# hila-chefer/Transformer-Explainability

Measured on NVIDIA H100. Metric: explanations_per_sec, higher is better.
Workload: dtype f32

## Files before the change

### transformer_explainability_b200/csrc/te_tc_wgmma.cu

```cuda
#include <cuda.h>
#include <cuda_bf16.h>
#include <cuda_fp16.h>
#include <cuda_runtime.h>
#include <string.h>
#include <algorithm>
#include <string>
#include <type_traits>
#include <utility>

#include "te_gemm_tc.h"
#include "te_wgmma.cuh"

namespace {

constexpr int BM = 128, NTHREADS = 256;

__device__ __forceinline__ uint32_t smem_u32(const void* p) { return (uint32_t)__cvta_generic_to_shared(p); }
__device__ __forceinline__ void fence_proxy_async() { asm volatile("fence.proxy.async.shared::cta;" ::: "memory"); }
__device__ __forceinline__ void wg_fence() { asm volatile("wgmma.fence.sync.aligned;" ::: "memory"); }
__device__ __forceinline__ void wg_commit() { asm volatile("wgmma.commit_group.sync.aligned;" ::: "memory"); }
__device__ __forceinline__ void wg_wait0() { asm volatile("wgmma.wait_group.sync.aligned 0;" ::: "memory"); }
__device__ __forceinline__ void wg_wait1() { asm volatile("wgmma.wait_group.sync.aligned 1;" ::: "memory"); }

__device__ __forceinline__ void mbar_init(uint32_t bar, uint32_t count) {
    asm volatile("mbarrier.init.shared::cta.b64 [%0], %1;" ::"r"(bar), "r"(count) : "memory");
}
__device__ __forceinline__ void mbar_expect_tx(uint32_t bar, uint32_t bytes) {
    asm volatile("mbarrier.arrive.expect_tx.shared::cta.b64 _, [%0], %1;" ::"r"(bar), "r"(bytes) : "memory");
}
__device__ __forceinline__ void mbar_arrive(uint32_t bar) { asm volatile("mbarrier.arrive.shared::cta.b64 _, [%0];" ::"r"(bar) : "memory"); }
__device__ __forceinline__ void mbar_wait(uint32_t bar, uint32_t parity) {
    uint32_t done;
    do {
        asm volatile("{\n.reg .pred p;\nmbarrier.try_wait.parity.shared::cta.b64 p, [%1], %2;\nselp.u32 %0, 1, 0, p;\n}\n"
                     : "=r"(done) : "r"(bar), "r"(parity) : "memory");
    } while (!done);
}
__device__ __forceinline__ void tma_load(uint32_t dst, const CUtensorMap* map, int k, int row, uint32_t bar) {
    asm volatile("cp.async.bulk.tensor.2d.shared::cluster.global.tile.mbarrier::complete_tx::bytes [%0], [%1, {%2, %3}], [%4];"
                 ::"r"(dst), "l"((uint64_t)map), "r"(k), "r"(row), "r"(bar) : "memory");
}
__device__ __forceinline__ void tma_load3(uint32_t dst, const CUtensorMap* map, int x, int y, int z, uint32_t bar) {
    asm volatile("cp.async.bulk.tensor.3d.shared::cluster.global.tile.mbarrier::complete_tx::bytes [%0], [%1, {%2, %3, %4}], [%5];"
                 ::"r"(dst), "l"((uint64_t)map), "r"(x), "r"(y), "r"(z), "r"(bar) : "memory");
}
__device__ __forceinline__ void bar_named(int id, int threads) { asm volatile("bar.sync %0, %1;" ::"r"(id), "r"(threads) : "memory"); }
template <int N>
__device__ __forceinline__ void setmaxnreg_dec() { asm volatile("setmaxnreg.dec.sync.aligned.u32 %0;" ::"n"(N)); }
template <int N>
__device__ __forceinline__ void setmaxnreg_inc() { asm volatile("setmaxnreg.inc.sync.aligned.u32 %0;" ::"n"(N)); }

__device__ __forceinline__ float to_tf32(float x) {
    uint32_t u;
    asm("cvt.rna.tf32.f32 %0, %1;" : "=r"(u) : "f"(x));
    return __uint_as_float(u);
}
__device__ __forceinline__ float4 tf32x4(float4 v) { return make_float4(to_tf32(v.x), to_tf32(v.y), to_tf32(v.z), to_tf32(v.w)); }
__device__ __forceinline__ float4 absx4(float4 v) { return make_float4(fabsf(v.x), fabsf(v.y), fabsf(v.z), fabsf(v.w)); }
__device__ __forceinline__ float4 posx4(float4 v) { return make_float4(fmaxf(v.x, 0.f), fmaxf(v.y, 0.f), fmaxf(v.z, 0.f), fmaxf(v.w, 0.f)); }
__device__ __forceinline__ float4 negx4(float4 v) { return make_float4(fminf(v.x, 0.f), fminf(v.y, 0.f), fminf(v.z, 0.f), fminf(v.w, 0.f)); }
__device__ __forceinline__ float4 subx4(float4 a, float4 b) { return make_float4(a.x - b.x, a.y - b.y, a.z - b.z, a.w - b.w); }

__device__ __forceinline__ float ex2_approx(float x) {
    float y;
    asm("ex2.approx.ftz.f32 %0, %1;" : "=f"(y) : "f"(x));
    return y;
}

__device__ __forceinline__ uint32_t swz(int r, int c) { return (uint32_t)r * 128u + ((uint32_t)(c ^ (r & 7)) << 4); }

// ... 117 lines not shown
}
template <bool SP>
__device__ __forceinline__ auto put_tf32(uint8_t* hi, uint8_t* lo) {
    return [=](int r, int c, float4 v) {
        if (SP) st4(hi, r, c, tf32x4(v));
        else st_split(hi, lo, r, c, v);
    };
}
template <bool SP>
__device__ __forceinline__ void fix_tf32(uint8_t* hi, uint8_t* lo, int r0, int n, int t, int nt) {
    if (SP) map_rows(hi, r0, n, t, nt, [](float4 v) { return tf32x4(v); });
    else split_rows(hi, lo, r0, n, t, nt);
}

__device__ __forceinline__ int frag_row(int tid, int j) { return 64 * (tid >> 7) + 16 * ((tid >> 5) & 3) + ((tid & 31) >> 2) + 8 * ((j >> 1) & 1); }
__device__ __forceinline__ int frag_col(int tid, int j) { return 8 * (j >> 2) + 2 * (tid & 3) + (j & 1); }

constexpr int TMA_MAPS = 5;
struct TmaArgs {
    CUtensorMap map[TMA_MAPS];
    int mtiles, ntiles, nz;
};
enum { FIX_NONE = 0, FIX_A = 1, FIX_AB = 2 };
constexpr int NTHREADS_TMA = 384, SMEM_MAX = 227 * 1024;
__host__ __device__ constexpr int tma_stages(int bytes, int epi) {
    return (SMEM_MAX - 1024 - 256 - epi) / bytes < 8 ? (SMEM_MAX - 1024 - 256 - epi) / bytes : 8;
}

template <class P>
__host__ __device__ constexpr int epi_bytes() { return P::EPI_MAPS * BM * P::BN * 4; }
__device__ __forceinline__ float2 epi_f2(const uint8_t* t, int r, int c) {
    return *reinterpret_cast<const float2*>(t + (c >> 5) * (BM * 128) + swz(r, (c & 31) >> 2) + (c & 3) * 4);
}

template <class P, int NA, int NR, int NT, int NTR>
__device__ __forceinline__ void fold(const P& p, float (&acc)[NA][NR], float (&tot)[NT][NTR], int m0, int ch, int z, int tid) {
    const float s0 = p.chunk_scale(m0 + frag_row(tid, 0), ch, z), s1 = p.chunk_scale(m0 + frag_row(tid, 2), ch, z);
#pragma unroll
    for (int a = 0; a < NA; ++a)
#pragma unroll
        for (int j = 0; j < NR; ++j) tot[a][j] = fmaf(acc[a][j], ((j >> 1) & 1) ? s1 : s0, tot[a][j]);
}
template <int NA, int NR>
__device__ __forceinline__ void zero(float (&v)[NA][NR]) {
#pragma unroll
    for (int a = 0; a < NA; ++a)
#pragma unroll
        for (int j = 0; j < NR; ++j) v[a][j] = 0.f;
}

template <class P>
__device__ __forceinline__ void reg_tile(const P& p, uint8_t* smem, int col_fast) {
    constexpr int NR = P::BN / 2;
    constexpr int NA = P::PRODS::NACC;
    constexpr int STAGE = P::L::BYTES;
    constexpr int NT = P::CHUNK ? NA : 1, NTR = P::CHUNK ? NR : 1;
    const int tid = threadIdx.x, wg = tid >> 7;
    const int m0 = (col_fast ? blockIdx.y : blockIdx.x) * BM, n0 = (col_fast ? blockIdx.x : blockIdx.y) * P::BN;
    const int z = blockIdx.z;
    float acc[NA][NR];
    float tot[NT][NTR];
    zero(acc);
    zero(tot);

    const int kb = p.kblocks();
    p.load(smem, 0, m0, n0, z, tid);
    fence_proxy_async();
    __syncthreads();
    for (int it = 0; it < kb; ++it) {
        const bool fresh = P::CHUNK ? (it % P::CHUNK == 0) : (it == 0);
        wg_fence();
        issue<P>(smem_u32(smem + (it & 1) * STAGE), wg, acc, fresh ? 0u : 1u);
        wg_commit();
        if (it + 1 < kb) p.load(smem + ((it + 1) & 1) * STAGE, it + 1, m0, n0, z, tid);
        wg_wait0();
        if constexpr (P::CHUNK > 0)
            if ((it + 1) % P::CHUNK == 0 || it + 1 == kb) fold(p, acc, tot, m0, it / P::CHUNK, z, tid);
        fence_proxy_async();
        __syncthreads();
    }
    if constexpr (P::CHUNK > 0) p.epilogue(tot, m0, n0, z, tid, nullptr);
    else p.epilogue(acc, m0, n0, z, tid, nullptr);
}

template <class P>
__device__ __forceinline__ void tma_tiles(const P& p, const TmaArgs& ta, uint8_t* smem) {
    using L = typename P::L;
    constexpr int NR = P::BN / 2;
    constexpr int NA = P::PRODS::NACC;
    constexpr int STAGE = L::BYTES, EPI = epi_bytes<P>(), S = tma_stages(STAGE, EPI);
    constexpr int NT = P::CHUNK ? NA : 1, NTR = P::CHUNK ? NR : 1;
    static_assert(S >= 2, "a TMA problem needs two stages");
    __shared__ __align__(8) uint64_t bars[2 * S + 2];
    const int tid = threadIdx.x, wg = tid >> 7;
    const uint32_t full0 = smem_u32(bars), empty0 = full0 + 8u * S, st0 = smem_u32(smem);
    const uint32_t efull = full0 + 16u * S, eempty = efull + 8u, ebuf = st0 + (uint32_t)S * STAGE;
    if (tid == 0) {
        for (int s = 0; s < S; ++s) {
            mbar_init(full0 + 8u * s, 1);
            mbar_init(empty0 + 8u * s, 8);
        }
        mbar_init(efull, 1);
        mbar_init(eempty, 8);
        asm volatile("fence.mbarrier_init.release.cluster;" ::: "memory");
    }
    __syncthreads();
    const int kb = p.kblocks(), per_z = ta.mtiles * ta.ntiles, ntiles = ta.nz * per_z;
    int stage = 0;
    uint32_t phase = 0;
    auto decode = [&](int t, int& m0, int& n0, int& z) {
        z = t / per_z;
        const int r = t - z * per_z;
        m0 = (r / ta.ntiles) * BM;
        n0 = (r % ta.ntiles) * P::BN;
    };

    if (wg == 2) {
        setmaxnreg_dec<40>();
        if (tid != 2 * 128) return;
        uint32_t ephase = 0;
        for (int t = blockIdx.x; t < ntiles; t += gridDim.x) {
            int m0, n0, z;
            decode(t, m0, n0, z);
            for (int it = 0; it < kb; ++it) {
                mbar_wait(empty0 + 8u * stage, phase ^ 1u);
                p.produce(ta, st0 + (uint32_t)stage * STAGE, full0 + 8u * stage, it, m0, n0, z);
                if (++stage == S) { stage = 0; phase ^= 1u; }
                if constexpr (EPI > 0) {
                    if (it == min(S, kb) - 1) {
                        mbar_wait(eempty, ephase ^ 1u);
                        mbar_expect_tx(efull, EPI);
#pragma unroll
                        for (int i = 0; i < P::EPI_MAPS; ++i)
#pragma unroll
                            for (int b = 0; b < P::BN / 32; ++b)
                                tma_load(ebuf + (uint32_t)(i * BM * P::BN * 4 + b * BM * 128), &ta.map[P::NMAPS + i], n0 + 32 * b,
                                         m0, efull);
                        ephase ^= 1u;
                    }
                }
            }
        }
        return;
    }

    setmaxnreg_inc<232>();
    float acc[NA][NR];
    float tot[NT][NTR];
    auto release = [&](int s) {
        if ((tid & 31) == 0) mbar_arrive(empty0 + 8u * s);
    };
    auto consume = [&](uint32_t sd) {
        mbar_wait(full0 + 8u * stage, phase);
        if constexpr (P::FIX != FIX_NONE) {
            p.fix(smem + (uint32_t)stage * STAGE, wg, tid);
            fence_proxy_async();
            if constexpr (P::FIX == FIX_A) bar_named(1 + wg, 128);
            else bar_named(3, 256);
        }
        wg_fence();
        issue<P>(st0 + (uint32_t)stage * STAGE, wg, acc, sd);
        wg_commit();
    };
    auto next = [&] {
        if (++stage == S) { stage = 0; phase ^= 1u; }
    };
    constexpr int CH = P::CHUNK;
    uint32_t ephase = 0;
    for (int t = blockIdx.x; t < ntiles; t += gridDim.x) {
        int m0, n0, z;
        decode(t, m0, n0, z);
        zero(acc);
        zero(tot);
        for (int k0 = 0; k0 < kb; k0 += CH ? CH : kb) {
            const int k1 = CH ? min(k0 + CH, kb) : kb;
            consume(0u);
            for (int it = k0 + 1; it < k1; ++it) {
                const int prev = stage;
                next();
                consume(1u);
                wg_wait1();
                release(prev);
            }
            wg_wait0();
            release(stage);
            next();
            if constexpr (CH > 0) fold(p, acc, tot, m0, k0 / CH, z, tid);
        }
        if constexpr (EPI > 0) mbar_wait(efull, ephase);
        if constexpr (P::CHUNK > 0) p.epilogue(tot, m0, n0, z, tid, smem + (uint32_t)S * STAGE);
        else p.epilogue(acc, m0, n0, z, tid, smem + (uint32_t)S * STAGE);
        if constexpr (EPI > 0) {
            __syncwarp();
            if ((tid & 31) == 0) mbar_arrive(eempty);
            ephase ^= 1u;
        }
    }
}

template <class P>
__global__ void __launch_bounds__(P::TMA ? NTHREADS_TMA : NTHREADS, 1)
    wg_kernel(const P p, const __grid_constant__ TmaArgs ta, int col_fast) {
    extern __shared__ uint8_t smem_raw[];
    uint8_t* smem = smem_raw + ((1024u - (smem_u32(smem_raw) & 1023u)) & 1023u);
    if constexpr (P::TMA) tma_tiles(p, ta, smem);
    else reg_tile(p, smem, col_fast);
}

struct NoScale {
    __device__ __forceinline__ float chunk_scale(int, int, int) const { return 1.f; }
};

struct TmaTile {
    const void* base;
    long long rows, cols, ld;
    int box_rows;
    long long count = 0, cstride = 0;
};
template <class P>
__device__ __forceinline__ void produce_tiles(const TmaArgs& ta, uint32_t st, uint32_t bar, int it, int m0, int n0) {
    using L = typename P::L;
    constexpr int KE = P::FMT == OP_TF32 ? 32 : 64;
    mbar_expect_tx(bar, L::BYTES);
#pragma unroll
    for (int i = 0; i < L::NTA; ++i) tma_load(st + L::a(i), &ta.map[i], it * KE, m0, bar);
#pragma unroll
    for (int j = 0; j < L::NTB; ++j) tma_load(st + L::b(j), &ta.map[L::NTA + j], it * KE, n0, bar);
}
#define TE_PRODUCE_TILES(P)                                                                                      \
    static constexpr int NMAPS = L::NTA + L::NTB;                                                                \
    __device__ void produce(const TmaArgs& ta, uint32_t st, uint32_t bar, int it, int m0, int n0, int) const { \
        produce_tiles<P>(ta, st, bar, it, m0, n0);                                                               \
    }

enum { ZO_F32 = 0, ZO_BF16 = 1, ZO_F16S = 2 };
template <bool SINGLE, bool BF, int OUT>
struct ZsProb : NoScale {
    static constexpr int BN = 128, CHUNK = 0, FMT = BF ? OP_BF16 : OP_TF32;
    using PRODS = std::conditional_t<SINGLE, One, Prods<Pr<0, 0, 0>, Pr<0, 1, 1>>>;
    using L = Stage<PRODS, BN>;
    static constexpr bool COL_FAST = true;
    static constexpr bool TMA = SINGLE;
    static constexpr int FIX = SINGLE && !BF ? FIX_A : FIX_NONE;
    static constexpr int EPI_MAPS = SINGLE ? 2 : 0;
    int M, N, K;
    const float* x; long long ldx;
    const void* xabs;
    const void* wa; const void* wb;
    const float* r; long long ldr; const float* y; long long ldy; const float* bias;
    void* out; long long ldo; float* hs;
    float sscale, zsign;

    __device__ int kblocks() const { return K / (BF ? 64 : 32); }
    __device__ void fix(uint8_t* st, int wg, int tid) const {
        map_rows(st + L::a(0), 64 * wg, 64, tid & 127, 128, [](float4 v) { return tf32x4(absx4(v)); });
    }
    TE_PRODUCE_TILES(ZsProb)
    TmaTile tile(int i) const {
        if (i == 0) return BF ? TmaTile{xabs, M, K, K, BM} : TmaTile{x, M, K, ldx, BM};
        if (i == 1) return TmaTile{wa, N, K, K, BN};
        return i == 2 ? TmaTile{r, M, N, ldr, BM} : TmaTile{y, M, N, ldy, BM};
    }
    __device__ void load(uint8_t* st, int kb, int m0, int n0, int, int tid) const {
        for_k32(BM, x, ldx, m0, M, kb * 32, K, tid, [&](int rr, int c, float4 v) {
            st4(st + L::a(0), rr, c, tf32x4(posx4(v)));
            st4(st + L::a(1), rr, c, tf32x4(negx4(v)));
        });
        for_k32(BN, (const float*)wa, K, n0, N, kb * 32, K, tid, [&](int rr, int c, float4 v) { st4(st + L::b(0), rr, c, v); });
        for_k32(BN, (const float*)wb, K, n0, N, kb * 32, K, tid, [&](int rr, int c, float4 v) { st4(st + L::b(1), rr, c, v); });
    }
    __device__ void epilogue(float (&acc)[1][BN / 2], int m0, int n0, int, int tid, const uint8_t* eb) const {
        float sv[BN / 2];
        float rmax[2] = {0.f, 0.f};
#pragma unroll
        for (int j = 0; j < BN / 2; j += 2) {
            const int row = m0 + frag_row(tid, j), col = n0 + frag_col(tid, j);
            float2 rr = make_float2(0.f, 0.f), z = make_float2(acc[0][j], acc[0][j + 1]);
            if (row < M) {
                rr = SINGLE ? epi_f2(eb, frag_row(tid, j), frag_col(tid, j))
                            : *reinterpret_cast<const float2*>(r + (long long)row * ldr + col);
                if (SINGLE) {
                    const float2 yy = epi_f2(eb + BM * BN * 4, frag_row(tid, j), frag_col(tid, j));
                    const float2 bb = bias ? *reinterpret_cast<const float2*>(bias + col) : make_float2(0.f, 0.f);
                    z.x = 0.5f * ((yy.x - bb.x) + zsign * z.x);
                    z.y = 0.5f * ((yy.y - bb.y) + zsign * z.y);
                    z = zsign > 0.f ? make_float2(fmaxf(z.x, 0.f), fmaxf(z.y, 0.f)) : make_float2(fminf(z.x, 0.f), fminf(z.y, 0.f));
                }
            }
            sv[j] = sscale * te_sd(rr.x, z.x);
            sv[j + 1] = sscale * te_sd(rr.y, z.y);
            if (OUT == ZO_F16S) rmax[(j >> 1) & 1] = fmaxf(rmax[(j >> 1) & 1], fmaxf(fabsf(sv[j]), fabsf(sv[j + 1])));
        }
#pragma unroll
        for (int j = 0; j < BN / 2; j += 2) {
            const int row = m0 + frag_row(tid, j), col = n0 + frag_col(tid, j);
            if (row >= M) continue;
            if (OUT == ZO_F32) {
                *reinterpret_cast<float2*>((float*)out + (long long)row * ldo + col) = make_float2(to_tf32(sv[j]), to_tf32(sv[j + 1]));
            } else if (OUT == ZO_BF16) {
                *reinterpret_cast<__nv_bfloat162*>((__nv_bfloat16*)out + (long long)row * ldo + col) = __floats2bfloat162_rn(sv[j], sv[j + 1]);
            }
        }
        if (OUT == ZO_F16S) {
            float sc[2];
#pragma unroll
            for (int h = 0; h < 2; ++h) {
                float m = rmax[h];
                m = fmaxf(m, __shfl_xor_sync(0xffffffffu, m, 1));
                m = fmaxf(m, __shfl_xor_sync(0xffffffffu, m, 2));
                float si;
                te_f16_block_scale(m, sc[h], si);
                const int row = m0 + frag_row(tid, 2 * h);
                if ((tid & 3) == 0 && row < M) hs[(long long)row * (N / 128) + n0 / 128] = si;
            }
#pragma unroll
            for (int j = 0; j < BN / 2; j += 2) {
                const int row = m0 + frag_row(tid, j), col = n0 + frag_col(tid, j);
                const float s = sc[(j >> 1) & 1];
                if (row < M) *reinterpret_cast<__half2*>((__half*)out + (long long)row * N + col) = __floats2half2_rn(sv[j] * s, sv[j + 1] * s);
            }
        }
    }
};

template <int KIND>
struct ZrProb {
    static constexpr int BN = (KIND == 2) ? 64 : 128, CHUNK = (KIND == 2) ? 2 : 0;
    static constexpr int FMT = KIND == 0 ? OP_TF32 : KIND == 1 ? OP_BF16 : OP_F16;
    using PRODS = Prods<Pr<0, 0, 0>, Pr<1, 0, 1>>;
    using L = Stage<PRODS, BN>;
    static constexpr bool TMA = true;
    static constexpr int FIX = FIX_NONE, EPI_MAPS = KIND == 0 ? 0 : 1;
    int M, N, K;
    const void* s; const void* wp; const void* wn;
    const float* rs; int rs_ld; const float* cp; const float* cn;
    const float* x; long long ldx; float* out; long long ldo;
    int accum;

    __device__ int kblocks() const { return K / (KIND ? 64 : 32); }
    TE_PRODUCE_TILES(ZrProb)
    __device__ float chunk_scale(int row, int ch, int) const { return (KIND == 2 && row < M) ? rs[(long long)row * rs_ld + ch] : 1.f; }
    TmaTile tile(int i) const {
        if (i == 0) return TmaTile{s, M, K, K, BM};
        return i < 3 ? TmaTile{i == 1 ? wp : wn, N, K, K, BN} : TmaTile{x, M, N, ldx, BM};
    }
    __device__ void epilogue(float (&acc)[2][BN / 2], int m0, int n0, int, int tid, const uint8_t* eb) const {
#pragma unroll
        for (int j = 0; j < BN / 2; j += 2) {
            const int row = m0 + frag_row(tid, j), col = n0 + frag_col(tid, j);
            if (row >= M) continue;
            const float2 xv = EPI_MAPS ? epi_f2(eb, frag_row(tid, j), frag_col(tid, j))
                                       : *reinterpret_cast<const float2*>(x + (long long)row * ldx + col);
            float2 ap = make_float2(acc[0][j], acc[0][j + 1]), an = make_float2(acc[1][j], acc[1][j + 1]);
            if (KIND == 2) {
                ap.x *= cp[col]; ap.y *= cp[col + 1];
                an.x *= cn[col]; an.y *= cn[col + 1];
            }
            float2 v = make_float2(fmaxf(xv.x, 0.f) * ap.x + fminf(xv.x, 0.f) * an.x, fmaxf(xv.y, 0.f) * ap.y + fminf(xv.y, 0.f) * an.y);
            if (accum) {
                const float2 prev = *reinterpret_cast<const float2*>(out + (long long)row * ldo + col);
                v = make_float2(prev.x + v.x, prev.y + v.y);
            }
            acc[0][j] = v.x;
            acc[0][j + 1] = v.y;
        }
// ... 8 lines not shown
template <bool NEG>
struct LrpSProb : NoScale {
    static constexpr int BN = 128, CHUNK = 0, FMT = OP_TF32;
    using PRODS = One;
    using L = Stage<PRODS, BN>;
    static constexpr bool COL_FAST = true, TMA = false;
    int M, N, K;
    const float* x; long long ldx; const float* w;
    const float* r; long long ldr; float* out;
    float sscale;
    __device__ int kblocks() const { return K / 32; }
    __device__ void load(uint8_t* st, int kb, int m0, int n0, int, int tid) const {
        for_k32(BM, x, ldx, m0, M, kb * 32, K, tid, [&](int rr, int c, float4 v) { st4(st + L::a(0), rr, c, tf32x4(NEG ? negx4(v) : posx4(v))); });
        for_k32(BN, w, K, n0, N, kb * 32, K, tid, [&](int rr, int c, float4 v) { st4(st + L::b(0), rr, c, v); });
    }
    __device__ void epilogue(float (&acc)[1][BN / 2], int m0, int n0, int, int tid, const uint8_t*) const {
#pragma unroll
        for (int j = 0; j < BN / 2; j += 2) {
            const int row = m0 + frag_row(tid, j), col = n0 + frag_col(tid, j);
            if (row >= M) continue;
            const float2 rr = *reinterpret_cast<const float2*>(r + (long long)row * ldr + col);
            *reinterpret_cast<float2*>(out + (long long)row * N + col) =
                make_float2(to_tf32(sscale * te_sd(rr.x, acc[0][j])), to_tf32(sscale * te_sd(rr.y, acc[0][j + 1])));
        }
    }
};
template <bool NEG>
struct LrpRProb : NoScale {
    static constexpr int BN = 128, CHUNK = 0, FMT = OP_TF32;
    using PRODS = One;
    using L = Stage<PRODS, BN>;
    static constexpr bool TMA = true;
    static constexpr int FIX = FIX_NONE, EPI_MAPS = 1;
    int M, N, K;
    const float* s; const float* wt;
    const float* x; long long ldx; float* out; long long ldo;
    int accum;
    __device__ int kblocks() const { return K / 32; }
    TE_PRODUCE_TILES(LrpRProb)
    TmaTile tile(int i) const {
        return i == 0 ? TmaTile{s, M, K, K, BM} : i == 1 ? TmaTile{wt, N, K, K, BN} : TmaTile{x, M, N, ldx, BM};
    }
    __device__ void epilogue(float (&acc)[1][BN / 2], int m0, int n0, int, int tid, const uint8_t* eb) const {
#pragma unroll
        for (int j = 0; j < BN / 2; j += 2) {
            const int row = m0 + frag_row(tid, j), col = n0 + frag_col(tid, j);
            if (row >= M) continue;
            const float2 xv = epi_f2(eb, frag_row(tid, j), frag_col(tid, j));
            const float2* o = reinterpret_cast<const float2*>(out + (long long)row * ldo + col);
            float2 v;
            if (NEG) {
                const float2 prev = *o;
                v = make_float2(prev.x + fminf(xv.x, 0.f) * acc[0][j], prev.y + fminf(xv.y, 0.f) * acc[0][j + 1]);
            } else if (accum) {
                const float2 prev = *o;
                v = make_float2(prev.x + fmaxf(xv.x, 0.f) * acc[0][j], prev.y + fmaxf(xv.y, 0.f) * acc[0][j + 1]);
            } else {
                v = make_float2(fmaxf(xv.x, 0.f) * acc[0][j], fmaxf(xv.y, 0.f) * acc[0][j + 1]);
            }
            acc[0][j] = v.x;
            acc[0][j + 1] = v.y;
        }
#pragma unroll
        for (int j = 0; j < BN / 2; j += 2) {
            const int row = m0 + frag_row(tid, j), col = n0 + frag_col(tid, j);
            if (row < M) *reinterpret_cast<float2*>(out + (long long)row * ldo + col) = make_float2(acc[0][j], acc[0][j + 1]);
// ... 20 lines not shown
}
template <int EPI, class EF>
__device__ __forceinline__ void lin_store(const LinOut& o, int row, int col, float2 y, EF e) {
    *reinterpret_cast<float2*>(o.C + (long long)row * o.ldc + col) = y;
    float2 y2 = make_float2(0.f, 0.f);
    if (EPI == TE_TC_EPI_BIAS_GELU) y2 = make_float2(te_gelu(y.x), te_gelu(y.y));
    if (EPI == TE_TC_EPI_BIAS_ADD) {
        const float2 ev = e();
        y2 = make_float2(ev.x + y.x, ev.y + y.y);
    }
    if (EPI == TE_TC_EPI_BIAS_GELU || EPI == TE_TC_EPI_BIAS_ADD) *reinterpret_cast<float2*>(o.C2 + (long long)row * o.ldc2 + col) = y2;
}

enum { LIN_3XTF32 = 0, LIN_TF32 = 1, LIN_F16X3 = 2, LIN_F16 = 3 };
struct LinArgs {
    int K, rs_ld;
    const void* a; const void* a_lo; long long lda;
    const void* b; const void* b_lo;
    const float* rs; const float* cs;
    LinOut o;
};
static_assert(sizeof(LinArgs) <= 128, "LinArgs: keep the kernel parameter within 128 bytes");
template <int EPI, int FORM>
struct LinProb : LinArgs {
    static constexpr bool F16 = FORM == LIN_F16X3 || FORM == LIN_F16, SPLIT = FORM == LIN_3XTF32 || FORM == LIN_F16X3;
    static constexpr int BN = FORM == LIN_TF32 && EPI == TE_TC_EPI_STORE ? 256 : 128;
    static constexpr int CHUNK = F16 ? 2 : SPLIT ? 4 : 0, FMT = F16 ? OP_F16 : OP_TF32;
    using PRODS = std::conditional_t<SPLIT, Split3, One>;
    using L = Stage<PRODS, BN>;
    static constexpr bool COL_FAST = true;
    static constexpr bool TMA = FORM != LIN_3XTF32;
    static constexpr int FIX = FORM == LIN_TF32 ? FIX_A : FIX_NONE;
    static constexpr int EPI_MAPS = TMA && EPI == TE_TC_EPI_GELU_BWD ? 1 : 0;
    __device__ int kblocks() const { return K / (F16 ? 64 : 32); }
    __device__ float chunk_scale(int row, int ch, int) const {
        if constexpr (F16) return row < o.M ? rs[(long long)row * rs_ld + ch] : 1.f;
        else return 1.f;
    }
    __device__ void fix(uint8_t* st, int wg, int tid) const {
        map_rows(st + L::a(0), 64 * wg, 64, tid & 127, 128, [](float4 v) { return tf32x4(v); });
    }
    TE_PRODUCE_TILES(LinProb)
    TmaTile tile(int i) const {
        if (i < L::NTA) return TmaTile{i == 0 ? a : a_lo, o.M, K, F16 ? K : lda, BM};
        if (i < NMAPS) return TmaTile{i == L::NTA ? b : b_lo, o.N, K, K, BN};
        return TmaTile{o.E, o.M, o.N, o.lde, BM};
    }
    __device__ void load(uint8_t* st, int kb, int m0, int n0, int, int tid) const {
        for_k32(BM, (const float*)a, lda, m0, o.M, kb * 32, K, tid, [&](int r, int c, float4 v) { st_split(st + L::a(0), st + L::a(1), r, c, v); });
        for_k32(BN, (const float*)b, K, n0, o.N, kb * 32, K, tid, [&](int r, int c, float4 v) { st4(st + L::b(0), r, c, v); });
        for_k32(BN, (const float*)b_lo, K, n0, o.N, kb * 32, K, tid, [&](int r, int c, float4 v) { st4(st + L::b(1), r, c, v); });
    }
    __device__ void epilogue(float (&acc)[1][BN / 2], int m0, int n0, int, int tid, const uint8_t* eb) const {
        auto inside = [&](int row, int col) { return row < o.M && (BN == 128 || col < o.N); };
        constexpr bool E_FIRST = EPI == TE_TC_EPI_BIAS_ADD && EPI_MAPS == 0;
        float2 ef[E_FIRST ? BN / 4 : 1];
#pragma unroll
        for (int j = 0; j < BN / 2; j += 2) {
            const int row = m0 + frag_row(tid, j), col = n0 + frag_col(tid, j);
            if (!inside(row, col)) continue;
            if constexpr (E_FIRST) ef[j / 2] = efrag(eb, tid, j, row, col);
            auto e = [&] { return efrag(eb, tid, j, row, col); };
            float2 y;
            if constexpr (F16)
                y = lin_value<EPI, false>(o, col, acc[0][j] * cs[col], acc[0][j + 1] * cs[col + 1], e);
            else y = lin_value<EPI, FORM == LIN_TF32>(o, col, acc[0][j], acc[0][j + 1], e);
            acc[0][j] = y.x;
            acc[0][j + 1] = y.y;
        }
#pragma unroll
        for (int j = 0; j < BN / 2; j += 2) {
            const int row = m0 + frag_row(tid, j), col = n0 + frag_col(tid, j);
            if (inside(row, col))
                lin_store<EPI>(o, row, col, make_float2(acc[0][j], acc[0][j + 1]), [&] {
                    if constexpr (E_FIRST) return ef[j / 2];
                    else return efrag(eb, tid, j, row, col);
                });
        }
    }
    __device__ float2 efrag(const uint8_t* eb, int tid, int j, int row, int col) const {
        if constexpr (EPI_MAPS > 0) return epi_f2(eb, frag_row(tid, j), frag_col(tid, j));
        else return *reinterpret_cast<const float2*>(o.E + (long long)row * o.lde + col);
    }
};

enum { AT_STORE = 0, AT_MUL = 1, AT_SD = 2, AT_SOFTMAX = 3, AT_RESID = 4 };
template <int EPI, bool SP, int BN_>
struct NnProb : NoScale {
    static constexpr int BN = BN_, CHUNK = 0, FMT = OP_TF32;
    using PRODS = std::conditional_t<SP, One, Split3>;
    using L = Stage<PRODS, BN>;
    static constexpr bool TMA = true;
    static constexpr int FIX = FIX_AB, EPI_MAPS = 0;
    int N, H, dh, ld_out, batch;
    const float* a; long long lda; const float* b; long long ldb;
    const float* E; float* out; float alpha;
    __device__ int kblocks() const { return dh / 32; }
    static constexpr int NMAPS = 2;
    TmaTile tile(int i) const {
        return i == 0 ? TmaTile{a, (long long)batch * N, H * dh, lda, BM} : TmaTile{b, (long long)batch * N, H * dh, ldb, BN};
    }
    __device__ void produce(const TmaArgs& ta, uint32_t st, uint32_t bar, int kb, int m0, int n0, int bh) const {
        const int s = bh / H, k = (bh % H) * dh + kb * 32;
        mbar_expect_tx(bar, TILE128 + BN * 128);
        tma_load(st + L::a(0), &ta.map[0], k, s * N + m0, bar);
        tma_load(st + L::b(0), &ta.map[1], k, s * N + n0, bar);
    }
    __device__ void fix(uint8_t* st, int wg, int tid) const {
        fix_tf32<SP>(st + L::a(0), st + L::a(1), 64 * wg, 64, tid & 127, 128);
        fix_tf32<SP>(st + L::b(0), st + L::b(1), 0, BN, tid, 256);
    }
    __device__ void epilogue(float (&acc)[1][BN / 2], int m0, int n0, int bh, int tid, const uint8_t*) const {
        const int ncols = (N + 3) & ~3;
        if constexpr (EPI == AT_SOFTMAX) {
            float mx[2] = {-INFINITY, -INFINITY};
#pragma unroll
            for (int j = 0; j < BN / 2; ++j)
                if (n0 + frag_col(tid, j) < N) mx[(j >> 1) & 1] = fmaxf(mx[(j >> 1) & 1], alpha * acc[0][j]);
            float sum[2] = {0.f, 0.f}, m2[2];
#pragma unroll
            for (int h = 0; h < 2; ++h) {
                mx[h] = fmaxf(mx[h], __shfl_xor_sync(0xffffffffu, mx[h], 1));
                mx[h] = fmaxf(mx[h], __shfl_xor_sync(0xffffffffu, mx[h], 2));
                m2[h] = -mx[h] * 1.4426950408889634f;
            }
            const float a2 = alpha * 1.4426950408889634f;
// ... 22 lines not shown
        for (int j = 0; j < BN / 2; j += 2) {
            const int r = m0 + frag_row(tid, j), col = n0 + frag_col(tid, j);
            ef[j / 2] = (EPI != AT_STORE && r < N && col < ncols)
                            ? *reinterpret_cast<const float2*>(E + ((long long)bh * N + r) * ld_out + col) : make_float2(0.f, 0.f);
        }
#pragma unroll
        for (int j = 0; j < BN / 2; j += 2) {
            const int r = m0 + frag_row(tid, j), col = n0 + frag_col(tid, j);
            if (r >= N || col >= ncols) continue;
            const long long off = ((long long)bh * N + r) * ld_out + col;
            const float2 e = ef[j / 2];
            float v[2] = {alpha * acc[0][j], alpha * acc[0][j + 1]};
            const float ee[2] = {e.x, e.y};
#pragma unroll
            for (int u = 0; u < 2; ++u) {
                if (EPI == AT_MUL) v[u] *= ee[u];
                else if (EPI == AT_SD) v[u] = te_sd_fast(ee[u], v[u]);
                if (col + u >= N) v[u] = 0.f;
            }
            *reinterpret_cast<float2*>(out + off) = make_float2(v[0], v[1]);
        }
        }
    }
};

template <int AMN, int EPI, bool SP, int BN_>
struct NkProb : NoScale {
    static constexpr int BN = BN_, CHUNK = SP ? 0 : 4, FMT = OP_TF32;
    using PRODS = std::conditional_t<SP, One, Split3>;
    static constexpr int LAND_A = AMN ? BM * 128 : 0, LAND_X = BN * 128;
    using L = Stage<PRODS, BN, LAND_A + LAND_X>;
    static constexpr bool TMA = true;
    static constexpr int FIX = FIX_AB, EPI_MAPS = 0;
    int N, H, NP, ld_out, n_out, n_pad, a_shared, batch;
    const float* map; const float* X; long long ldx;
    const float* rowscale; const float* E; float* out; float alpha;
    __device__ int kblocks() const { return (N + 31) / 32; }
    static constexpr int NMAPS = 2;
    TmaTile tile(int i) const {
        if (i == 0) return TmaTile{map, N, N, NP, AMN ? 32 : BM, (long long)batch * (a_shared ? 1 : H), (long long)N * NP};
        return TmaTile{X, N, n_pad, ldx, 32, batch, (long long)N * ldx};
    }
    __device__ void produce(const TmaArgs& ta, uint32_t st, uint32_t bar, int kb, int m0, int, int bh) const {
        const int s = bh / H, h = bh % H, za = a_shared ? s : bh;
        mbar_expect_tx(bar, (AMN ? LAND_A : TILE128) + LAND_X);
        if (AMN == 0) tma_load3(st + L::a(0), &ta.map[0], kb * 32, m0, za, bar);
#pragma unroll
        for (int j = 0; j < LAND_A / 4096; ++j) tma_load3(st + L::land() + j * 4096, &ta.map[0], m0 + 32 * j, kb * 32, za, bar);
#pragma unroll
        for (int j = 0; j < LAND_X / 4096; ++j)
            tma_load3(st + L::land() + LAND_A + j * 4096, &ta.map[1], h * BN + 32 * j, kb * 32, s, bar);
    }
    __device__ void fix(uint8_t* st, int wg, int tid) const {
        if (AMN) transpose_rows(st + L::land(), 64 * wg, 64, tid & 127, 128, put_tf32<SP>(st + L::a(0), st + L::a(1)));
        else fix_tf32<SP>(st + L::a(0), st + L::a(1), 64 * wg, 64, tid & 127, 128);
        transpose_rows(st + L::land() + LAND_A, 0, BN, tid, 256, put_tf32<SP>(st + L::b(0), st + L::b(1)));
    }
    __device__ void epilogue(float (&acc)[1][BN / 2], int m0, int, int bh, int tid, const uint8_t*) const {
        const int s = bh / H, h = bh % H;
        float2 ef[BN / 4];
#pragma unroll
        for (int j = 0; j < BN / 2; j += 2) {
            const int m = m0 + frag_row(tid, j), gcol = h * BN + frag_col(tid, j);
            ef[j / 2] = (EPI != AT_STORE && m < N && gcol < n_pad)
                            ? *reinterpret_cast<const float2*>(E + ((long long)s * N + m) * ld_out + gcol) : make_float2(0.f, 0.f);
        }
// ... 32 lines not shown
                                 const cuuint32_t*, const cuuint32_t*, CUtensorMapInterleave, CUtensorMapSwizzle,
                                 CUtensorMapL2promotion, CUtensorMapFloatOOBfill);
EncodeTiled encode_tiled() {
    static const EncodeTiled fn = [] {
        void* f = nullptr;
        cudaDriverEntryPointQueryResult q;
        if (cudaGetDriverEntryPoint("cuTensorMapEncodeTiled", &f, cudaEnableDefault, &q) != cudaSuccess ||
            q != cudaDriverEntryPointSuccess)
            return (EncodeTiled) nullptr;
        return (EncodeTiled)f;
    }();
    return fn;
}
bool encode_tile(CUtensorMap* map, const TmaTile& t, int esize) {
    const EncodeTiled fn = encode_tiled();
    const int rank = t.count > 0 ? 3 : 2;
    if (!fn || ((uintptr_t)t.base & 15u) || (t.ld * esize) % 16 != 0 || (t.cstride * esize) % 16 != 0 || t.rows < 1 || t.cols < 1)
        return false;
    const cuuint64_t dims[3] = {(cuuint64_t)t.cols, (cuuint64_t)t.rows, (cuuint64_t)t.count};
    const cuuint64_t strides[2] = {(cuuint64_t)(t.ld * esize), (cuuint64_t)(t.cstride * esize)};
    const cuuint32_t box[3] = {(cuuint32_t)(128 / esize), (cuuint32_t)t.box_rows, 1}, estr[3] = {1, 1, 1};
    return fn(map, esize == 4 ? CU_TENSOR_MAP_DATA_TYPE_FLOAT32 : CU_TENSOR_MAP_DATA_TYPE_UINT16, rank, const_cast<void*>(t.base),
              dims, strides, box, estr, CU_TENSOR_MAP_INTERLEAVE_NONE, CU_TENSOR_MAP_SWIZZLE_128B,
              CU_TENSOR_MAP_L2_PROMOTION_L2_256B, CU_TENSOR_MAP_FLOAT_OOB_FILL_NONE) == CUDA_SUCCESS;
}

template <class P>
int launch(const P& p, dim3 grid, cudaStream_t st) {
    TmaArgs ta;
    memset(&ta, 0, sizeof(ta));
    int col_fast = 0, threads = NTHREADS, smem = 2 * P::L::BYTES + 1024;
    if constexpr (P::TMA) {
        constexpr int ESIZE = P::FMT == OP_TF32 ? 4 : 2;
        static_assert(P::NMAPS + P::EPI_MAPS <= TMA_MAPS, "TmaArgs holds TMA_MAPS tensor maps");
        for (int i = 0; i < P::NMAPS + P::EPI_MAPS; ++i)
            if (!encode_tile(&ta.map[i], p.tile(i), i < P::NMAPS ? ESIZE : 4)) {
                te_set_last_error("te_tc: cannot encode a TMA tensor map (16-byte-aligned base and strides required)");
                return TE_ERR_ARG;
            }
        const long long tiles = (long long)grid.x * grid.y * grid.z;
        if (tiles > INT32_MAX) { te_set_last_error("te_tc: grid too large for one launch"); return TE_ERR_ARG; }
        ta.mtiles = (int)grid.x;
        ta.ntiles = (int)grid.y;
        ta.nz = (int)grid.z;
        grid = dim3((unsigned)std::min<long long>(tiles, sm_count()));
        threads = NTHREADS_TMA;
        smem = tma_stages(P::L::BYTES, epi_bytes<P>()) * P::L::BYTES + epi_bytes<P>() + 1024;
    } else {
        col_fast = P::COL_FAST && grid.x <= 65535;
        if (col_fast) grid = dim3(grid.y, grid.x, grid.z);
    }
    static unsigned long long done = 0;
    int dev = 0;
    if (cudaGetDevice(&dev) != cudaSuccess) { te_set_last_error("te_tc: cudaGetDevice failed"); return TE_ERR_CUDA; }
    if (!(done & (1ull << (dev & 63)))) {
        if (cudaFuncSetAttribute(wg_kernel<P>, cudaFuncAttributeMaxDynamicSharedMemorySize, smem) != cudaSuccess) {
            te_set_last_error("te_tc: cannot raise dynamic shared memory");
            return TE_ERR_CUDA;
        }
        done |= 1ull << (dev & 63);
    }
    if (grid.y > 65535 || grid.z > 65535) { te_set_last_error("te_tc: grid too large for one launch"); return TE_ERR_ARG; }
    wg_kernel<P><<<grid, threads, smem, st>>>(p, ta, col_fast);
    TE_CUDA_CHECK_LAUNCH();
    return TE_OK;
}
inline unsigned mtiles(long long M) { return (unsigned)((M + BM - 1) / BM); }

__global__ void prepare_weights_kernel(const float* __restrict__ w, float* __restrict__ d, int out_f, int in_f) {
    const TeDerived<float> dv(d, in_f, out_f);
    __shared__ float tile[32][33];
    const int bx = blockIdx.x * 32, by = blockIdx.y * 32;
    for (int i = threadIdx.y; i < 32; i += blockDim.y) {
        const int o = by + i, c = bx + threadIdx.x;
        float v = 0.f;
        if (o < out_f && c < in_f) {
            const long long idx = (long long)o * in_f + c;
            v = w[idx];
            dv.wp[idx] = to_tf32(fmaxf(v, 0.f));
            dv.wn[idx] = to_tf32(fminf(v, 0.f));
// ... 150 lines not shown

int te_tc_rowsplit_f16(const float* x, long long ldx, long long rows, int cols, void* hi, void* lo, float* scale_inv,
                       cudaStream_t st) {
    if (cols % 4 != 0 || ldx % 4 != 0 || !a16(x) || ((uintptr_t)hi & 7u) || (lo && ((uintptr_t)lo & 7u))) {
        te_set_last_error("te_tc_rowsplit_f16: alignment");
        return TE_ERR_ARG;
    }
    rowsplit_f16_kernel<<<stride_blocks(rows, 8), 256, 0, st>>>(x, ldx, rows, cols / 4, reinterpret_cast<__half*>(hi),
                                                                reinterpret_cast<__half*>(lo), scale_inv);
    TE_CUDA_CHECK_LAUNCH();
    return TE_OK;
}

int te_tc_blocksplit_f16(const float* x, long long ldx, long long rows, int cols, float* split, float* scale_inv, cudaStream_t st,
                         bool hi_only) {
    if (cols % 4 != 0 || ldx % 4 != 0 || !a16(x) || !a16(split) || !scale_inv) {
        te_set_last_error("te_tc_blocksplit_f16: alignment");
        return TE_ERR_ARG;
    }
    __half* hi = reinterpret_cast<__half*>(split);
    blocksplit_f16_kernel<<<stride_blocks(rows, 8), 256, 0, st>>>(x, ldx, rows, cols, hi, hi_only ? nullptr : hi + rows * cols,
                                                                  scale_inv);
    TE_CUDA_CHECK_LAUNCH();
    return TE_OK;
}

bool te_tc_zplus_supported(long long rows, int in_features, int out_features, long long ldx) {
    return rows > 0 && rows < (1LL << 31) && in_features % 128 == 0 && out_features % 128 == 0 && ldx % 4 == 0;
}
int te_tc_zplus_s1(const float* x, long long ldx, float* xabs, const float* derived, const float* r, long long ldr,
                   const float* y, long long ldy, const float* bias, float* s_out, long long rows, int in_features,
                   int out_features, cudaStream_t st, bool bf16, float* s16, float* s16_scale, float s_scale, bool inh) {
    const TeDerived<const float> dv(derived, in_features, out_features);
    if (ldx % 4 != 0 || !a16(x) || !a16(r) || !a16(y) || ldr % 4 != 0 || ldy % 4 != 0) {
        te_set_last_error("te_tc_zplus_s1: alignment");
        return TE_ERR_ARG;
    }
    void* o = s16 ? (void*)s16 : (void*)s_out;
    auto run = [&](auto zs_fn, const void* wa) {
        return zs_fn(x, ldx, xabs, wa, nullptr, r, ldr, y, ldy, bias, o, s16_scale, rows, in_features, out_features, st, s_scale,
                     inh);
    };
    if (bf16 && in_features % 64 == 0) {
        if (!a16(xabs)) { te_set_last_error("te_tc_zplus_s1: alignment"); return TE_ERR_ARG; }
        abs_bf16_kernel<<<stride_blocks(rows * (in_features / 4), 256), 256, 0, st>>>(
            x, ldx, reinterpret_cast<__nv_bfloat16*>(xabs), rows, in_features / 4);
        TE_CUDA_CHECK_LAUNCH();
        return s16 ? run(zs<true, true, ZO_F16S>, dv.bf_wabs) : run(zs<true, true, ZO_F32>, dv.bf_wabs);
    }
    return s16 ? run(zs<true, false, ZO_F16S>, dv.wabs) : run(zs<true, false, ZO_F32>, dv.wabs);
}

int te_tc_zplus_r(const float* s, const float* derived, const float* x, long long ldx, float* out, long long ld_out,
                  long long rows, int in_features, int out_features, cudaStream_t st, bool inh) {
    const TeDerived<const float> dv(derived, in_features, out_features);
    ZrProb<0> p;
    memset(&p, 0, sizeof(p));
    p.M = (int)rows; p.N = in_features; p.K = out_features;
    p.s = s; p.wp = inh ? dv.wnt : dv.wpt; p.wn = inh ? dv.wpt : dv.wnt; p.x = x; p.ldx = ldx; p.out = out; p.ldo = ld_out;
    p.accum = inh;
    return launch(p, dim3(mtiles(rows), in_features / 128), st);
}

int te_tc_zplus_r16(const float* s, float* split, float* scale, const float* derived, const float* x, long long ldx, float* out,
                    long long ld_out, long long rows, int in_features, int out_features, cudaStream_t st, bool inh) {
    const TeDerived<const float> dv(derived, in_features, out_features);
    if (!a16(split) || !scale || !a16(derived) || !a16(x) || !a16(out) || ldx % 4 != 0 || ld_out % 4 != 0) {
// ... 237 lines not shown
```

Before: 923.3.

## Stream epilogue operands through a slot ring and write results with TMA stores

Replaces the single whole-tile epilogue buffer with a ring of 32-column slots. The producer warp feeds the ring opportunistically between mainloop loads, which frees shared memory for more mainloop stages and lets epilogue loads overlap compute. For the f32 z-plus and GELU-backward linear paths, results are written back into the slot and sent to global memory with bulk TMA tensor stores instead of per-thread stores. This adds barrier and phase bookkeeping, an extra tensor map and an alignment requirement on the output.

```diff
diff --git a/transformer_explainability_b200/csrc/te_tc_wgmma.cu b/transformer_explainability_b200/csrc/te_tc_wgmma.cu
--- a/transformer_explainability_b200/csrc/te_tc_wgmma.cu
+++ b/transformer_explainability_b200/csrc/te_tc_wgmma.cu
@@ -36,6 +36,26 @@
                      : "=r"(done) : "r"(bar), "r"(parity) : "memory");
     } while (!done);
 }
+__device__ __forceinline__ bool mbar_test(uint32_t bar, uint32_t parity) {
+    uint32_t done;
+    asm volatile("{\n.reg .pred p;\nmbarrier.test_wait.parity.shared::cta.b64 p, [%1], %2;\nselp.u32 %0, 1, 0, p;\n}\n"
+                 : "=r"(done) : "r"(bar), "r"(parity) : "memory");
+    return done != 0;
+}
+__device__ __forceinline__ bool mbar_try(uint32_t bar, uint32_t parity) {
+    uint32_t done;
+    asm volatile("{\n.reg .pred p;\nmbarrier.try_wait.parity.shared::cta.b64 p, [%1], %2, 100;\nselp.u32 %0, 1, 0, p;\n}\n"
+                 : "=r"(done) : "r"(bar), "r"(parity) : "memory");
+    return done != 0;
+}
+__device__ __forceinline__ void tma_store(const CUtensorMap* map, uint32_t src, int col, int row) {
+    asm volatile("cp.async.bulk.tensor.2d.global.shared::cta.bulk_group [%0, {%2, %3}], [%1];"
+                 ::"l"((uint64_t)map), "r"(src), "r"(col), "r"(row) : "memory");
+}
+__device__ __forceinline__ void bulk_commit() { asm volatile("cp.async.bulk.commit_group;" ::: "memory"); }
+template <int N>
+__device__ __forceinline__ void bulk_wait_read() { asm volatile("cp.async.bulk.wait_group.read %0;" ::"n"(N) : "memory"); }
+__device__ __forceinline__ void bulk_wait_all() { asm volatile("cp.async.bulk.wait_group 0;" ::: "memory"); }
 __device__ __forceinline__ void tma_load(uint32_t dst, const CUtensorMap* map, int k, int row, uint32_t bar) {
     asm volatile("cp.async.bulk.tensor.2d.shared::cluster.global.tile.mbarrier::complete_tx::bytes [%0], [%1, {%2, %3}], [%4];"
                  ::"r"(dst), "l"((uint64_t)map), "r"(k), "r"(row), "r"(bar) : "memory");
@@ -219,6 +239,60 @@
 __device__ __forceinline__ float2 epi_f2(const uint8_t* t, int r, int c) {
     return *reinterpret_cast<const float2*>(t + (c >> 5) * (BM * 128) + swz(r, (c & 31) >> 2) + (c & 3) * 4);
 }
+__device__ __forceinline__ void epi_st2(uint8_t* t, int r, int c, float2 v) {
+    *reinterpret_cast<float2*>(t + (c >> 5) * (BM * 128) + swz(r, (c & 31) >> 2) + (c & 3) * 4) = v;
+}
+
+template <class P>
+struct Smem {
+    static constexpr int STAGE = P::L::BYTES, SLOT = P::RING ? P::EPI_MAPS * BM * 128 : 0, EPI = P::RING ? 0 : epi_bytes<P>();
+    static constexpr int S = tma_stages(STAGE, P::RING ? P::RING_MIN * SLOT : EPI);
+    static constexpr int FREE = SMEM_MAX - 1024 - 256 - S * STAGE;
+    static constexpr int ESLOTS = !P::RING ? 0 : FREE / SLOT < P::BN / 32 ? FREE / SLOT : P::BN / 32;
+    static constexpr int BYTES = S * STAGE + EPI + ESLOTS * SLOT;
+};
+
+template <int ES, bool TSTORE>
+struct EpiRing {
+    uint32_t full0, empty0, base;
+    uint8_t* base_ptr;
+    int slot_bytes, slot = 0;
+    uint32_t phase = 0, pending = 0;
+    __device__ __forceinline__ uint8_t* wait() {
+        mbar_wait(full0 + 8u * slot, phase);
+        return base_ptr + slot * slot_bytes;
+    }
+    __device__ __forceinline__ void next() {
+        if (++slot == ES) { slot = 0; phase ^= 1u; }
+    }
+    __device__ __forceinline__ void release(int tid) {
+        __syncwarp();
+        if ((tid & 31) == 0) mbar_arrive(empty0 + 8u * slot);
+        next();
+    }
+    __device__ __forceinline__ void store(const CUtensorMap* map, int col, int row0, int tid) {
+        const int wg = tid >> 7;
+        fence_proxy_async();
+        bar_named(1 + wg, 128);
+        if ((tid & 127) == 0) {
+            tma_store(map, base + (uint32_t)(slot * slot_bytes + wg * 64 * 128), col, row0 + 64 * wg);
+            bulk_commit();
+            if (pending) {
+                bulk_wait_read<1>();
+                mbar_arrive(pending);
+            }
+            pending = empty0 + 8u * slot;
+        }
+        next();
+    }
+    __device__ __forceinline__ void flush(int tid) {
+        if ((tid & 127) == 0 && pending) {
+            bulk_wait_read<0>();
+            mbar_arrive(pending);
+            pending = 0;
+        }
+    }
+};
 
 template <class P, int NA, int NR, int NT, int NTR>
 __device__ __forceinline__ void fold(const P& p, float (&acc)[NA][NR], float (&tot)[NT][NTR], int m0, int ch, int z, int tid) {
@@ -273,22 +347,27 @@
 template <class P>
 __device__ __forceinline__ void tma_tiles(const P& p, const TmaArgs& ta, uint8_t* smem) {
     using L = typename P::L;
+    using SM = Smem<P>;
     constexpr int NR = P::BN / 2;
     constexpr int NA = P::PRODS::NACC;
-    constexpr int STAGE = L::BYTES, EPI = epi_bytes<P>(), S = tma_stages(STAGE, EPI);
+    constexpr int STAGE = L::BYTES, EPI = SM::EPI, S = SM::S, ES = SM::ESLOTS;
     constexpr int NT = P::CHUNK ? NA : 1, NTR = P::CHUNK ? NR : 1;
     static_assert(S >= 2, "a TMA problem needs two stages");
-    __shared__ __align__(8) uint64_t bars[2 * S + 2];
+    static_assert(!P::RING || ES >= 2, "the epilogue ring needs two slots");
+    static_assert(!P::TSTORE || P::RING, "TMA stores go through the ring");
+    __shared__ __align__(8) uint64_t bars[2 * S + (P::RING ? 2 * ES : 2)];
     const int tid = threadIdx.x, wg = tid >> 7;
     const uint32_t full0 = smem_u32(bars), empty0 = full0 + 8u * S, st0 = smem_u32(smem);
-    const uint32_t efull = full0 + 16u * S, eempty = efull + 8u, ebuf = st0 + (uint32_t)S * STAGE;
+    const uint32_t efull = full0 + 16u * S, eempty = efull + 8u * (P::RING ? ES : 1), ebuf = st0 + (uint32_t)S * STAGE;
     if (tid == 0) {
         for (int s = 0; s < S; ++s) {
             mbar_init(full0 + 8u * s, 1);
             mbar_init(empty0 + 8u * s, 8);
         }
-        mbar_init(efull, 1);
-        mbar_init(eempty, 8);
+        for (int s = 0; s < (P::RING ? ES : 1); ++s) {
+            mbar_init(efull + 8u * s, 1);
+            mbar_init(eempty + 8u * s, P::TSTORE ? 2 : 8);
+        }
         asm volatile("fence.mbarrier_init.release.cluster;" ::: "memory");
     }
     __syncthreads();
@@ -306,13 +385,34 @@
         setmaxnreg_dec<40>();
         if (tid != 2 * 128) return;
         uint32_t ephase = 0;
+        int et = blockIdx.x, ec = 0, es = 0, ready = -1;
+        auto feed = [&] {
+            while (et < ntiles && et <= ready && mbar_test(eempty + 8u * es, ephase ^ 1u)) {
+                int m0, n0, z;
+                decode(et, m0, n0, z);
+                const uint32_t f = efull + 8u * es, dst = ebuf + (uint32_t)(es * SM::SLOT);
+                mbar_expect_tx(f, SM::SLOT);
+#pragma unroll
+                for (int i = 0; i < P::EPI_MAPS; ++i) tma_load(dst + (uint32_t)(i * BM * 128), &ta.map[P::NMAPS + i], n0 + 32 * ec, m0, f);
+                if (++es == ES) { es = 0; ephase ^= 1u; }
+                if (++ec == P::BN / 32) { ec = 0; et += gridDim.x; }
+            }
+        };
         for (int t = blockIdx.x; t < ntiles; t += gridDim.x) {
             int m0, n0, z;
             decode(t, m0, n0, z);
             for (int it = 0; it < kb; ++it) {
-                mbar_wait(empty0 + 8u * stage, phase ^ 1u);
+                if constexpr (P::RING) {
+                    while (!mbar_try(empty0 + 8u * stage, phase ^ 1u)) feed();
+                } else {
+                    mbar_wait(empty0 + 8u * stage, phase ^ 1u);
+                }
                 p.produce(ta, st0 + (uint32_t)stage * STAGE, full0 + 8u * stage, it, m0, n0, z);
                 if (++stage == S) { stage = 0; phase ^= 1u; }
+                if constexpr (P::RING) {
+                    if (it == min(S, kb) - 1) ready = t;
+                    feed();
+                }
                 if constexpr (EPI > 0) {
                     if (it == min(S, kb) - 1) {
                         mbar_wait(eempty, ephase ^ 1u);
@@ -326,6 +426,12 @@
                         ephase ^= 1u;
                     }
                 }
+            }
+        }
+        if constexpr (P::RING) {
+            while (et < ntiles) {
+                mbar_wait(eempty + 8u * es, ephase ^ 1u);
+                feed();
             }
         }
         return;
@@ -354,6 +460,7 @@
     };
     constexpr int CH = P::CHUNK;
     uint32_t ephase = 0;
+    EpiRing<P::RING ? ES : 1, P::TSTORE> ring{efull, eempty, ebuf, smem + (uint32_t)S * STAGE, SM::SLOT};
     for (int t = blockIdx.x; t < ntiles; t += gridDim.x) {
         int m0, n0, z;
         decode(t, m0, n0, z);
@@ -374,6 +481,11 @@
             next();
             if constexpr (CH > 0) fold(p, acc, tot, m0, k0 / CH, z, tid);
         }
+        if constexpr (P::RING) {
+            if constexpr (P::CHUNK > 0) p.epilogue_ring(tot, m0, n0, z, tid, ring, ta);
+            else p.epilogue_ring(acc, m0, n0, z, tid, ring, ta);
+            continue;
+        }
         if constexpr (EPI > 0) mbar_wait(efull, ephase);
         if constexpr (P::CHUNK > 0) p.epilogue(tot, m0, n0, z, tid, smem + (uint32_t)S * STAGE);
         else p.epilogue(acc, m0, n0, z, tid, smem + (uint32_t)S * STAGE);
@@ -383,6 +495,8 @@
             ephase ^= 1u;
         }
     }
+    if constexpr (P::TSTORE)
+        if ((tid & 127) == 0) bulk_wait_all();
 }
 
 template <class P>
@@ -430,6 +544,8 @@
     static constexpr bool TMA = SINGLE;
     static constexpr int FIX = SINGLE && !BF ? FIX_A : FIX_NONE;
     static constexpr int EPI_MAPS = SINGLE ? 2 : 0;
+    static constexpr bool RING = SINGLE, TSTORE = SINGLE && OUT == ZO_F32;
+    static constexpr int RING_MIN = 3;
     int M, N, K;
     const float* x; long long ldx;
     const void* xabs;
@@ -446,6 +562,7 @@
     TmaTile tile(int i) const {
         if (i == 0) return BF ? TmaTile{xabs, M, K, K, BM} : TmaTile{x, M, K, ldx, BM};
         if (i == 1) return TmaTile{wa, N, K, K, BN};
+        if (i == 4) return TmaTile{out, M, N, ldo, 64};
         return i == 2 ? TmaTile{r, M, N, ldr, BM} : TmaTile{y, M, N, ldy, BM};
     }
     __device__ void load(uint8_t* st, int kb, int m0, int n0, int, int tid) const {
@@ -456,28 +573,53 @@
         for_k32(BN, (const float*)wa, K, n0, N, kb * 32, K, tid, [&](int rr, int c, float4 v) { st4(st + L::b(0), rr, c, v); });
         for_k32(BN, (const float*)wb, K, n0, N, kb * 32, K, tid, [&](int rr, int c, float4 v) { st4(st + L::b(1), rr, c, v); });
     }
-    __device__ void epilogue(float (&acc)[1][BN / 2], int m0, int n0, int, int tid, const uint8_t* eb) const {
+    __device__ __forceinline__ float2 s2(float2 rr, float2 z, float2 yy, float2 bb) const {
+        if (SINGLE) {
+            z.x = 0.5f * ((yy.x - bb.x) + zsign * z.x);
+            z.y = 0.5f * ((yy.y - bb.y) + zsign * z.y);
+            z = zsign > 0.f ? make_float2(fmaxf(z.x, 0.f), fmaxf(z.y, 0.f)) : make_float2(fminf(z.x, 0.f), fminf(z.y, 0.f));
+        }
+        return make_float2(sscale * te_sd(rr.x, z.x), sscale * te_sd(rr.y, z.y));
+    }
+    __device__ void epilogue(float (&acc)[1][BN / 2], int m0, int n0, int, int tid, const uint8_t*) const {
         float sv[BN / 2];
         float rmax[2] = {0.f, 0.f};
 #pragma unroll
         for (int j = 0; j < BN / 2; j += 2) {
             const int row = m0 + frag_row(tid, j), col = n0 + frag_col(tid, j);
-            float2 rr = make_float2(0.f, 0.f), z = make_float2(acc[0][j], acc[0][j + 1]);
-            if (row < M) {
-                rr = SINGLE ? epi_f2(eb, frag_row(tid, j), frag_col(tid, j))
-                            : *reinterpret_cast<const float2*>(r + (long long)row * ldr + col);
-                if (SINGLE) {
-                    const float2 yy = epi_f2(eb + BM * BN * 4, frag_row(tid, j), frag_col(tid, j));
-                    const float2 bb = bias ? *reinterpret_cast<const float2*>(bias + col) : make_float2(0.f, 0.f);
-                    z.x = 0.5f * ((yy.x - bb.x) + zsign * z.x);
-                    z.y = 0.5f * ((yy.y - bb.y) + zsign * z.y);
-                    z = zsign > 0.f ? make_float2(fmaxf(z.x, 0.f), fmaxf(z.y, 0.f)) : make_float2(fminf(z.x, 0.f), fminf(z.y, 0.f));
-                }
-            }
-            sv[j] = sscale * te_sd(rr.x, z.x);
-            sv[j + 1] = sscale * te_sd(rr.y, z.y);
+            float2 rr = make_float2(0.f, 0.f);
+            if (row < M) rr = *reinterpret_cast<const float2*>(r + (long long)row * ldr + col);
+            const float2 s = s2(rr, make_float2(acc[0][j], acc[0][j + 1]), make_float2(0.f, 0.f), make_float2(0.f, 0.f));
+            sv[j] = s.x;
+            sv[j + 1] = s.y;
             if (OUT == ZO_F16S) rmax[(j >> 1) & 1] = fmaxf(rmax[(j >> 1) & 1], fmaxf(fabsf(sv[j]), fabsf(sv[j + 1])));
         }
+        store(sv, rmax, m0, n0, tid);
+    }
+    template <class RG>
+    __device__ void epilogue_ring(float (&acc)[1][BN / 2], int m0, int n0, int, int tid, RG& ring, const TmaArgs& ta) const {
+        float sv[BN / 2];
+        float rmax[2] = {0.f, 0.f};
+#pragma unroll
+        for (int c = 0; c < BN / 32; ++c) {
+            uint8_t* sl = ring.wait();
+#pragma unroll
+            for (int j = 16 * c; j < 16 * c + 16; j += 2) {
+                const int rl = frag_row(tid, j), cl = frag_col(tid, j) & 31, col = n0 + frag_col(tid, j);
+                const float2 bb = bias ? *reinterpret_cast<const float2*>(bias + col) : make_float2(0.f, 0.f);
+                const float2 s = s2(epi_f2(sl, rl, cl), make_float2(acc[0][j], acc[0][j + 1]), epi_f2(sl + BM * 128, rl, cl), bb);
+                sv[j] = s.x;
+                sv[j + 1] = s.y;
+                if (OUT == ZO_F16S) rmax[(j >> 1) & 1] = fmaxf(rmax[(j >> 1) & 1], fmaxf(fabsf(sv[j]), fabsf(sv[j + 1])));
+                if (OUT == ZO_F32) epi_st2(sl, rl, cl, make_float2(to_tf32(sv[j]), to_tf32(sv[j + 1])));
+            }
+            if constexpr (OUT == ZO_F32) ring.store(&ta.map[NMAPS + EPI_MAPS], n0 + 32 * c, m0, tid);
+            else ring.release(tid);
+        }
+        if constexpr (OUT == ZO_F32) ring.flush(tid);
+        else store(sv, rmax, m0, n0, tid);
+    }
+    __device__ void store(const float (&sv)[BN / 2], const float (&rmax)[2], int m0, int n0, int tid) const {
 #pragma unroll
         for (int j = 0; j < BN / 2; j += 2) {
             const int row = m0 + frag_row(tid, j), col = n0 + frag_col(tid, j);
@@ -518,6 +660,8 @@
     using L = Stage<PRODS, BN>;
     static constexpr bool TMA = true;
     static constexpr int FIX = FIX_NONE, EPI_MAPS = KIND == 0 ? 0 : 1;
+    static constexpr bool RING = false, TSTORE = false;
+    static constexpr int RING_MIN = 0;
     int M, N, K;
     const void* s; const void* wp; const void* wn;
     const float* rs; int rs_ld; const float* cp; const float* cn;
@@ -592,6 +736,8 @@
     using L = Stage<PRODS, BN>;
     static constexpr bool TMA = true;
     static constexpr int FIX = FIX_NONE, EPI_MAPS = 1;
+    static constexpr bool RING = false, TSTORE = false;
+    static constexpr int RING_MIN = 0;
     int M, N, K;
     const float* s; const float* wt;
     const float* x; long long ldx; float* out; long long ldo;
@@ -678,6 +824,8 @@
     static constexpr bool TMA = FORM != LIN_3XTF32;
     static constexpr int FIX = FORM == LIN_TF32 ? FIX_A : FIX_NONE;
     static constexpr int EPI_MAPS = TMA && EPI == TE_TC_EPI_GELU_BWD ? 1 : 0;
+    static constexpr bool RING = EPI_MAPS > 0, TSTORE = EPI_MAPS > 0;
+    static constexpr int RING_MIN = 4;
     __device__ int kblocks() const { return K / (F16 ? 64 : 32); }
     __device__ float chunk_scale(int row, int ch, int) const {
         if constexpr (F16) return row < o.M ? rs[(long long)row * rs_ld + ch] : 1.f;
@@ -690,7 +838,26 @@
     TmaTile tile(int i) const {
         if (i < L::NTA) return TmaTile{i == 0 ? a : a_lo, o.M, K, F16 ? K : lda, BM};
         if (i < NMAPS) return TmaTile{i == L::NTA ? b : b_lo, o.N, K, K, BN};
+        if (i == NMAPS + EPI_MAPS) return TmaTile{o.C, o.M, o.N, o.ldc, 64};
         return TmaTile{o.E, o.M, o.N, o.lde, BM};
+    }
+    template <class RG>
+    __device__ void epilogue_ring(float (&acc)[1][BN / 2], int m0, int n0, int, int tid, RG& ring, const TmaArgs& ta) const {
+#pragma unroll
+        for (int c = 0; c < BN / 32; ++c) {
+            uint8_t* sl = ring.wait();
+#pragma unroll
+            for (int j = 16 * c; j < 16 * c + 16; j += 2) {
+                const int rl = frag_row(tid, j), cl = frag_col(tid, j) & 31, col = n0 + frag_col(tid, j);
+                auto e = [&] { return epi_f2(sl, rl, cl); };
+                float2 y;
+                if constexpr (F16) y = lin_value<EPI, false>(o, col, acc[0][j] * cs[col], acc[0][j + 1] * cs[col + 1], e);
+                else y = lin_value<EPI, FORM == LIN_TF32>(o, col, acc[0][j], acc[0][j + 1], e);
+                epi_st2(sl, rl, cl, y);
+            }
+            ring.store(&ta.map[NMAPS + EPI_MAPS], n0 + 32 * c, m0, tid);
+        }
+        ring.flush(tid);
     }
     __device__ void load(uint8_t* st, int kb, int m0, int n0, int, int tid) const {
         for_k32(BM, (const float*)a, lda, m0, o.M, kb * 32, K, tid, [&](int r, int c, float4 v) { st_split(st + L::a(0), st + L::a(1), r, c, v); });
@@ -738,6 +905,8 @@
     using L = Stage<PRODS, BN>;
     static constexpr bool TMA = true;
     static constexpr int FIX = FIX_AB, EPI_MAPS = 0;
+    static constexpr bool RING = false, TSTORE = false;
+    static constexpr int RING_MIN = 0;
     int N, H, dh, ld_out, batch;
     const float* a; long long lda; const float* b; long long ldb;
     const float* E; float* out; float alpha;
@@ -826,6 +995,8 @@
     using L = Stage<PRODS, BN, LAND_A + LAND_X>;
     static constexpr bool TMA = true;
     static constexpr int FIX = FIX_AB, EPI_MAPS = 0;
+    static constexpr bool RING = false, TSTORE = false;
+    static constexpr int RING_MIN = 0;
     int N, H, NP, ld_out, n_out, n_pad, a_shared, batch;
     const float* map; const float* X; long long ldx;
     const float* rowscale; const float* E; float* out; float alpha;
@@ -924,8 +1095,9 @@
     int col_fast = 0, threads = NTHREADS, smem = 2 * P::L::BYTES + 1024;
     if constexpr (P::TMA) {
         constexpr int ESIZE = P::FMT == OP_TF32 ? 4 : 2;
-        static_assert(P::NMAPS + P::EPI_MAPS <= TMA_MAPS, "TmaArgs holds TMA_MAPS tensor maps");
-        for (int i = 0; i < P::NMAPS + P::EPI_MAPS; ++i)
+        constexpr int MAPS = P::NMAPS + P::EPI_MAPS + (P::TSTORE ? 1 : 0);
+        static_assert(MAPS <= TMA_MAPS, "TmaArgs holds TMA_MAPS tensor maps");
+        for (int i = 0; i < MAPS; ++i)
             if (!encode_tile(&ta.map[i], p.tile(i), i < P::NMAPS ? ESIZE : 4)) {
                 te_set_last_error("te_tc: cannot encode a TMA tensor map (16-byte-aligned base and strides required)");
                 return TE_ERR_ARG;
@@ -937,7 +1109,7 @@
         ta.nz = (int)grid.z;
         grid = dim3((unsigned)std::min<long long>(tiles, sm_count()));
         threads = NTHREADS_TMA;
-        smem = tma_stages(P::L::BYTES, epi_bytes<P>()) * P::L::BYTES + epi_bytes<P>() + 1024;
+        smem = Smem<P>::BYTES + 1024;
     } else {
         col_fast = P::COL_FAST && grid.x <= 65535;
         if (col_fast) grid = dim3(grid.y, grid.x, grid.z);
@@ -1154,7 +1326,7 @@
                    const float* y, long long ldy, const float* bias, float* s_out, long long rows, int in_features,
                    int out_features, cudaStream_t st, bool bf16, float* s16, float* s16_scale, float s_scale, bool inh) {
     const TeDerived<const float> dv(derived, in_features, out_features);
-    if (ldx % 4 != 0 || !a16(x) || !a16(r) || !a16(y) || ldr % 4 != 0 || ldy % 4 != 0) {
+    if (ldx % 4 != 0 || !a16(x) || !a16(r) || !a16(y) || ldr % 4 != 0 || ldy % 4 != 0 || (!s16 && !a16(s_out))) {
         te_set_last_error("te_tc_zplus_s1: alignment");
         return TE_ERR_ARG;
     }
```

New measurement: 947.5 (median of 6 runs). +2.6%, better.
